# dhansmair/flamingo-mini

Measured on AMD Instinct MI355X. Metric: images/sec (fwd+bwd) flamingo-mini bs=32, higher is better.
Workload: dtype bf16

## Files before the change

### flamingo-mini_amd/csrc/ff_gemm.hip

```cpp
#include <atomic>
#include <type_traits>
#include "ff_common.h"
#include <stdlib.h>
#include "ff_internal.h"
#include "ff_gemm_tiles.h"

namespace ff {

template <typename T>
FF_DEV void epilogue4(const GemmParams& P, const GemmProblem& pr, int m, int n, float (&v)[4]) {
    typedef __attribute__((ext_vector_type(4))) T vec4;
    const long long off = P.c_map.off(m) + n;
    const bool full = (n + 3 < P.N);
#pragma unroll
    for (int r = 0; r < 4; r++) v[r] *= P.scale;
    auto load4 = [&](const void* base, long long at, float (&o)[4]) {
        const T* p = (const T*)base + at;
        if (full) {
            vec4 t = *(const vec4*)p;
#pragma unroll
            for (int r = 0; r < 4; r++) o[r] = to_f32(t[r]);
        } else {
#pragma unroll
            for (int r = 0; r < 4; r++) o[r] = (n + r < P.N) ? to_f32(p[r]) : 0.f;
// ... 1057 lines not shown
    if (dtype == FF_DTYPE_BF16)
        return std::max(plan_bf16(M, N, K, nz, 0, 0, 0).split, plan_bf16(M, N, K, nz, 0, 0, 1).split);
    const long long tiles = (long long)cdiv(M, kFBM) * cdiv(N, kFBM) * nz;
    if (tiles >= 128 || K < 1024) return 1;
    int s = (int)(256 / tiles);
    s = std::min(s, K / 512);
    s = std::min(s, 16);
    return std::max(s, 1);
}

size_t gemm_workspace_bytes(int dtype, int M, int N, int K, int nz, int split_k) {
    if (split_k <= 0) split_k = gemm_pick_split(dtype, M, N, K, nz);
    return split_k > 1 ? (size_t)split_k * nz * M * N * sizeof(float) : 0;
}

int gemm_launch(GemmParams P, int dtype, void* workspace, size_t ws_bytes, hipStream_t st, int* leave_partial) {
    if (leave_partial) *leave_partial = 1;
    FF_CHECK(P.M > 0 && P.N > 0 && P.K > 0 && P.nz >= 1 && P.nz <= kGemmMaxZ, FF_ERR_SHAPE, "gemm: bad shape M=%d N=%d K=%d nz=%d",
             P.M, P.N, P.K, P.nz);
    P.tile = kFBM;
    if (dtype == FF_DTYPE_BF16) {
        const TilePlan plan = plan_bf16(P.M, P.N, P.K, P.nz, P.split_k, P.a_layout, P.b_layout, P.force_tile);
        P.tile = plan.tile;
        P.split_k = plan.split;
    } else if (P.split_k <= 0) P.split_k = gemm_pick_split(dtype, P.M, P.N, P.K, P.nz);
    const int kq = dtype == FF_DTYPE_BF16 ? kBK : kFBK;
    P.k_per_split = cdiv(cdiv(P.K, P.split_k), kq) * kq;
    P.split_k = cdiv(P.K, P.k_per_split);
    P.partial = nullptr;
    if (P.split_k > 1) {
        const size_t need = gemm_workspace_bytes(dtype, P.M, P.N, P.K, P.nz, P.split_k);
        FF_CHECK(workspace && ws_bytes >= need, FF_ERR_WORKSPACE, "gemm split-K workspace: need %zu have %zu", need, ws_bytes);
        FF_CHECK(P.N % 4 == 0, FF_ERR_UNSUPPORTED, "gemm split-K needs N %% 4 == 0 (N=%d)", P.N);
        P.partial = (float*)workspace;
    }
    {
        const int tm_edge = dtype == FF_DTYPE_BF16 ? (P.tile == 256128 || P.tile == 256256 ? 256 : P.tile == 128 || P.tile == 128160 || P.tile == 128002 ? 128 : P.tile == 3264 || P.tile == 3216 ? 32 : 64) : kFBM;
        const int tn_edge = dtype == FF_DTYPE_BF16 ? (P.tile == 3216 ? 16 : P.tile == 64 || P.tile == 64002 || P.tile == 3264 ? 64 : P.tile == 128160 ? 160 : P.tile == 256256 ? 256 : 128) : kFBM;
        const int tiles_m = cdiv(P.M, tm_edge), tiles_n = cdiv(P.N, tn_edge);
        double best = 1e300;
        P.xcd_ms = 1; P.xcd_ns = 1;
        for (int ms = 1; ms <= 8; ms *= 2) {
            const int ns = 8 / ms;
            if (ms > tiles_m || ns > tiles_n) continue;
            const double cost = (double)P.M / ms + (double)P.N / ns;
            if (cost < best) { best = cost; P.xcd_ms = ms; P.xcd_ns = ns; }
        }
        static const int disable = env_int("FF_GEMM_XCD2D", 1) == 0;
        if (disable) { P.xcd_ms = 1; P.xcd_ns = 1; }
    }
    const int vec = dtype == FF_DTYPE_BF16 ? 8 : 4;
    auto map_ok = [&](const RowMap& m) { return m.ld % vec == 0 && (m.rows_per_seg <= 0 || m.seg_stride % vec == 0); };
    const int a_contig = P.a_layout == 0 ? P.K : P.M, b_contig = P.b_layout == 0 ? P.K : P.N;
    P.a_vec_ok = map_ok(P.a_map) && a_contig % vec == 0;
    P.b_vec_ok = map_ok(P.b_map) && b_contig % vec == 0;
    for (int z = 0; z < P.nz; z++) {
        P.a_vec_ok = P.a_vec_ok && ((uintptr_t)P.p[z].A % 16 == 0);
        P.b_vec_ok = P.b_vec_ok && ((uintptr_t)P.p[z].B % 16 == 0);
    }
    P.c_vec8 = P.N % vec == 0 && map_ok(P.c_map) && map_ok(P.r_map);
    for (int z = 0; z < P.nz; z++)
        P.c_vec8 = P.c_vec8 && ((uintptr_t)P.p[z].C | (uintptr_t)P.p[z].aux_out | (uintptr_t)P.p[z].aux_in | (uintptr_t)P.p[z].residual) % 16 == 0;
    int rc;
    const int prof_id = prof_begin(P, dtype, P.tile, st);
    if (dtype == FF_DTYPE_BF16) {
        FF_CHECK(P.a_vec_ok && P.b_vec_ok, FF_ERR_UNSUPPORTED,
                 "bf16 gemm needs 16-byte aligned operands with contiguous dims %% 8 == 0 (M=%d N=%d K=%d)", P.M, P.N, P.K);
        FF_CHECK(P.N % 4 == 0 && P.c_map.ld % 4 == 0, FF_ERR_UNSUPPORTED, "bf16 gemm needs N %% 4 == 0 (N=%d)", P.N);
        auto span_ok = [&](const RowMap& m, int rows, int contig) {
            const long long last = (m.rows_per_seg > 0 ? (long long)((rows - 1) / m.rows_per_seg) * m.seg_stride + (long long)((rows - 1) % m.rows_per_seg) * m.ld
                                                      : (long long)(rows - 1) * m.ld) + contig;
            return last < (1LL << 30);
        };
        FF_CHECK(span_ok(P.a_map, P.a_layout == 0 ? P.M : P.K, a_contig) && span_ok(P.b_map, P.b_layout == 0 ? P.N : P.K, b_contig),
                 FF_ERR_UNSUPPORTED, "bf16 gemm operands must span < 2^30 elements (M=%d N=%d K=%d)", P.M, P.N, P.K);
        rc = run_bf16_dma(P, st);
    } else {
        rc = dispatch_f32(P, st);
    }
    prof_end(prof_id, st);
    FF_TRY(rc);
    if (P.split_k > 1 && leave_partial && P.nz == 1 && P.scale == 1.f && P.act < 0 && P.act_bwd < 0 && !P.p[0].aux_out && !P.p[0].gate &&
        !P.p[0].residual) {
        *leave_partial = P.split_k;
        return FF_OK;
    }
    if (P.split_k > 1) {
        const long long total = (long long)P.nz * P.M * ((P.N + 7) / 8);
        FF_CHECK(total < (1LL << 31), FF_ERR_UNSUPPORTED, "gemm split-K output too large (M=%d N=%d nz=%d)", P.M, P.N, P.nz);
        const int grid = (int)((total + 255) / 256);
        if (dtype == FF_DTYPE_BF16) hipLaunchKernelGGL(gemm_splitk_epilogue_kernel<bf16>, dim3(grid), dim3(256), 0, st, P);
        else hipLaunchKernelGGL(gemm_splitk_epilogue_kernel<float>, dim3(grid), dim3(256), 0, st, P);
        FF_TRY(check_launch("gemm_splitk_epilogue"));
    }
    return FF_OK;
}

}

#ifdef FF_GEMM_TIMELINE
extern "C" int ff_debug_timeline_read(unsigned long long* out, int n_blocks) {
    return (int)hipMemcpyFromSymbol(out, HIP_SYMBOL(ff::g_timeline), sizeof(unsigned long long) * 8 * n_blocks);
}
#endif

extern "C" size_t ff_gemm_workspace_bytes(const ff_gemm_desc* d) {
    int split = d->split_k;
    if (split <= 0 && d->tile > 0 && d->dtype == FF_DTYPE_BF16) split = ff::plan_bf16(d->M, d->N, d->K, 1, 0, d->a_layout, d->b_layout, d->tile).split;
    return ff::gemm_workspace_bytes(d->dtype, d->M, d->N, d->K, 1, split);
}

extern "C" int ff_gemm(const ff_gemm_desc* d, const void* A, const void* B, void* C, void* aux_out, const void* aux_in,
                       const void* residual, const void* gate, void* workspace, size_t workspace_bytes, ff_stream_t stream) {
    using namespace ff;
    FF_CHECK(d && A && B && C, FF_ERR_SHAPE, "ff_gemm: null argument");
    FF_CHECK(d->dtype == FF_DTYPE_F32 || d->dtype == FF_DTYPE_BF16, FF_ERR_UNSUPPORTED, "ff_gemm: dtype %d", d->dtype);
    FF_CHECK(d->act_bwd < 0 || aux_in, FF_ERR_SHAPE, "ff_gemm: act_bwd needs aux_in");
    GemmParams P = {};
    P.M = d->M; P.N = d->N; P.K = d->K;
    P.a_layout = d->a_layout; P.b_layout = d->b_layout;
// ... 56 lines not shown
```

### flamingo-mini_amd/csrc/ff_loss.hip

```cpp
#include "ff_common.h"
#include "ff_internal.h"

namespace ff {

template <typename T, typename F>
FF_DEV void for_row_vectors(const T* row, int V, F&& f) {
    constexpr int N = Vec<T>::N;
    int head = (int)(((16u - (unsigned)((unsigned long long)row & 15u)) & 15u) / sizeof(T));
    head = head < V ? head : V;
    const int nvec = (V - head) / N, tail0 = head + nvec * N;
    if ((int)threadIdx.x < head) f((int)threadIdx.x, to_f32(row[threadIdx.x]));
    for (int v = threadIdx.x; v < nvec; v += 256) {
        float x[N];
        Vec<T>::load(row + head + v * N, x);
#pragma unroll
        for (int e = 0; e < N; e++) f(head + v * N + e, x[e]);
    }
    for (int c = tail0 + threadIdx.x; c < V; c += 256) f(c, to_f32(row[c]));
}

template <typename T>
__global__ __launch_bounds__(256) void shifted_ce_fwd_kernel(int L, int V, const T* __restrict__ logits, const long long* __restrict__ labels,
                                                             long long ignore_index, float* __restrict__ loss_row, float* __restrict__ lse) {
    __shared__ float sm[4], ss[4];
// ... 5 lines not shown
        if (x > m) { s = s * __expf(m - x) + 1.f; m = x; }
        else s += __expf(x - m);
    });
#pragma unroll
    for (int o = 32; o > 0; o >>= 1) {
        const float m2 = __shfl_xor(m, o, 64), s2 = __shfl_xor(s, o, 64);
        const float mn = fmaxf(m, m2);
        s = (m == -INFINITY ? 0.f : s * __expf(m - mn)) + (m2 == -INFINITY ? 0.f : s2 * __expf(m2 - mn));
        m = mn;
    }
    const int w = threadIdx.x >> 6;
    if ((threadIdx.x & 63) == 0) { sm[w] = m; ss[w] = s; }
    __syncthreads();
    if (threadIdx.x == 0) {
        float M = fmaxf(fmaxf(sm[0], sm[1]), fmaxf(sm[2], sm[3])), S = 0.f;
        for (int k = 0; k < 4; k++) S += ss[k] * __expf(sm[k] - M);
        const float l = M + logf(S);
        lse[r] = l;
        const long long tgt = labels[(long long)b * L + i + 1];
        loss_row[r] = tgt == ignore_index ? 0.f : ((tgt < 0 || tgt >= V) ? __builtin_nanf("") : l - to_f32(row[tgt]));
    }
}

template <typename T>
__global__ __launch_bounds__(256) void shifted_ce_bwd_kernel(int L, int V, const T* __restrict__ logits, const long long* __restrict__ labels,
                                                             long long ignore_index, const float* __restrict__ lse, const float* __restrict__ g,
                                                             T* __restrict__ dlogits) {
    pin_args(L, V, logits, labels, ignore_index, lse, g, dlogits);
    const int b = blockIdx.x / L, i = blockIdx.x - b * L;
    const long long off = ((long long)b * L + i) * V;
    constexpr int N = Vec<T>::N;
    const T* row = logits + off;
    T* drow = dlogits + off;
    const bool last = i == L - 1;
    const int r = b * (L - 1) + i;
    const long long tgt = last ? -1 : labels[(long long)b * L + i + 1];
    const float gr = (last || tgt == ignore_index) ? 0.f : ((tgt < 0 || tgt >= V) ? __builtin_nanf("") : g[r]), l = last ? 0.f : lse[r];
    auto dval = [&](int c, float x) { return gr == 0.f ? 0.f : (__expf(x - l) - (c == tgt ? 1.f : 0.f)) * gr; };
    int head = (int)(((16u - (unsigned)((unsigned long long)row & 15u)) & 15u) / sizeof(T));
    head = head < V ? head : V;
    const int nvec = (V - head) / N, tail0 = head + nvec * N;
    if ((int)threadIdx.x < head) drow[threadIdx.x] = from_f32<T>(dval(threadIdx.x, to_f32(row[threadIdx.x])));
    for (int v = threadIdx.x; v < nvec; v += 256) {
        const int c0 = head + v * N;
        float x[N];
        Vec<T>::load(row + c0, x);
#pragma unroll
        for (int e = 0; e < N; e++) x[e] = dval(c0 + e, x[e]);
        Vec<T>::store(drow + c0, x);
    }
    for (int c = tail0 + threadIdx.x; c < V; c += 256) drow[c] = from_f32<T>(dval(c, to_f32(row[c])));
}

}

extern "C" int ff_shifted_ce_fwd(int dtype, int batch, int seq, int vocab, const void* logits, const long long* labels, long long ignore_index,
                                 float* loss_row, float* lse, ff_stream_t stream) {
    using namespace ff;
    FF_CHECK(batch > 0 && seq > 1 && vocab > 0 && logits && labels && loss_row && lse, FF_ERR_SHAPE, "ff_shifted_ce_fwd: bad arguments");
    const dim3 grid(batch * (seq - 1));
    if (dtype == FF_DTYPE_BF16) shifted_ce_fwd_kernel<bf16><<<grid, dim3(256), 0, (hipStream_t)stream>>>(seq, vocab, (const bf16*)logits, labels, ignore_index, loss_row, lse);
    else if (dtype == FF_DTYPE_F32) shifted_ce_fwd_kernel<float><<<grid, dim3(256), 0, (hipStream_t)stream>>>(seq, vocab, (const float*)logits, labels, ignore_index, loss_row, lse);
    else FF_CHECK(false, FF_ERR_UNSUPPORTED, "ff_shifted_ce_fwd: dtype %d", dtype);
    return check_launch("shifted_ce_fwd");
}

extern "C" int ff_shifted_ce_bwd(int dtype, int batch, int seq, int vocab, const void* logits, const long long* labels, long long ignore_index,
                                 const float* lse, const float* grad_row, void* dlogits, ff_stream_t stream) {
    using namespace ff;
    FF_CHECK(batch > 0 && seq > 1 && vocab > 0 && logits && labels && lse && grad_row && dlogits, FF_ERR_SHAPE, "ff_shifted_ce_bwd: bad arguments");
    FF_CHECK((((unsigned long long)logits ^ (unsigned long long)dlogits) & 15u) == 0, FF_ERR_UNSUPPORTED, "ff_shifted_ce_bwd: logits and dlogits must share their 16-byte alignment phase");
    const dim3 grid(batch * seq);
    if (dtype == FF_DTYPE_BF16) shifted_ce_bwd_kernel<bf16><<<grid, dim3(256), 0, (hipStream_t)stream>>>(seq, vocab, (const bf16*)logits, labels, ignore_index, lse, grad_row, (bf16*)dlogits);
    else if (dtype == FF_DTYPE_F32) shifted_ce_bwd_kernel<float><<<grid, dim3(256), 0, (hipStream_t)stream>>>(seq, vocab, (const float*)logits, labels, ignore_index, lse, grad_row, (float*)dlogits);
    else FF_CHECK(false, FF_ERR_UNSUPPORTED, "ff_shifted_ce_bwd: dtype %d", dtype);
    return check_launch("shifted_ce_bwd");
}
```

### flamingo-mini_amd/ffi.py

```python
from __future__ import annotations

import ctypes as C
import os
from typing import Optional, Sequence

import torch

PKG_DIR = os.path.dirname(os.path.abspath(__file__))
_which = os.environ.get("FLAMINGO_FUSION_LIB", "")
LIB_PATH = os.path.join(PKG_DIR, "libflamingo_fusion_debug.so") if _which == "debug" else (_which or os.path.join(PKG_DIR, "libflamingo_fusion.so"))
ABI_VERSION = 6

FF_OK = 0
DTYPE_F32, DTYPE_BF16 = 0, 1
ACT_NONE, ACT_GELU, ACT_SQRELU, ACT_RELU = -1, 0, 1, 2
ACTS = {"gelu": ACT_GELU, "sqrelu": ACT_SQRELU, "relu": ACT_RELU}
ATTN_DENSE, ATTN_MEDIA = 0, 1
RESAMPLER_GLOBAL_PARAMS, RESAMPLER_LAYER_PARAMS, XATTN_PARAMS = 4, 12, 11
WGRAD_GROUP_MAX = 12


class FusionLibraryError(RuntimeError):
    pass

# ... 55 lines not shown

class XattnDesc(C.Structure):
    _fields_ = [("dtype", C.c_int), ("batch", C.c_int), ("n_tokens", C.c_int), ("dim", C.c_int), ("dim_visual", C.c_int),
                ("n_media", C.c_int), ("n_visual", C.c_int), ("heads", C.c_int), ("dim_head", C.c_int), ("ff_mult", C.c_int),
                ("act", C.c_int), ("tt_stride", C.c_int), ("tt_offset", C.c_int), ("cached_k", Strides), ("cached_v", Strides),
                ("sync", C.c_void_p)]


_P, _SZ, _I = C.c_void_p, C.c_size_t, C.c_int
_SIGNATURES = {
    "ff_version": (_I, []),
    "ff_arch": (C.c_char_p, []),
    "ff_last_error": (C.c_char_p, []),
    "ff_gemm_workspace_bytes": (_SZ, [C.POINTER(GemmDesc)]),
    "ff_gemm": (_I, [C.POINTER(GemmDesc), _P, _P, _P, _P, _P, _P, _P, _P, _SZ, _P]),
    "ff_gemm_profile_enable": (_I, [_I]),
    "ff_gemm_profile_read": (_I, [C.POINTER(GemmProfileRecord), _I]),
    "ff_gemm_plan": (_I, [C.POINTER(GemmDesc), C.POINTER(_I), C.POINTER(_I), C.POINTER(_I)]),
    "ff_layernorm_fwd": (_I, [C.POINTER(LnDesc), _P, _P, _P, _P, _P, _P, _P, _P]),
    "ff_layernorm_bwd_workspace_bytes": (_SZ, [C.POINTER(LnDesc)]),
    "ff_layernorm_bwd": (_I, [C.POINTER(LnDesc), _P, _P, _P, _P, _P, _P, _P, _P, _P, _P, _P, _SZ, _P]),
    "ff_rows_reduce_workspace_bytes": (_SZ, [C.POINTER(ReduceDesc)]),
    "ff_rows_reduce": (_I, [C.POINTER(ReduceDesc), _P, _P, _P, _SZ, _P]),
    "ff_gate_grad_workspace_bytes": (_SZ, [_I, _I]),
    "ff_gate_grad": (_I, [_I, _I, _I, _P, _P, _P, _P, _P, _SZ, _P]),
    "ff_text_time": (_I, [_I, _I, _P, _I, _P, _P]),
    "ff_attention_fwd": (_I, [C.POINTER(AttnDesc), _P, _P, _P, _P, _P, _P, _P]),
    "ff_attention_bwd_workspace_bytes": (_SZ, [C.POINTER(AttnDesc)]),
    "ff_attention_bwd": (_I, [C.POINTER(AttnDesc), _P, _P, _P, _P, _P, _P, _P, _P, _P, _P, _P, _SZ, _P]),
    "ff_resampler_saved_bytes": (_SZ, [C.POINTER(ResamplerDesc)]),
    "ff_resampler_scratch_bytes": (_SZ, [C.POINTER(ResamplerDesc)]),
    "ff_resampler_fwd": (_I, [C.POINTER(ResamplerDesc), _P, _P, _P, _P, _SZ, _P, _SZ, _P]),
    "ff_resampler_bwd": (_I, [C.POINTER(ResamplerDesc), _P, _P, _P, _P, _SZ, _P, _P, _P, _SZ, _P]),
    "ff_resampler_prologue_saved_bytes": (_SZ, [C.POINTER(ResamplerDesc)]),
    "ff_resampler_layer_saved_bytes": (_SZ, [C.POINTER(ResamplerDesc)]),
    "ff_resampler_layer_scratch_bytes": (_SZ, [C.POINTER(ResamplerDesc)]),
    "ff_resampler_epilogue_saved_bytes": (_SZ, [C.POINTER(ResamplerDesc)]),
    "ff_resampler_prologue_fwd": (_I, [C.POINTER(ResamplerDesc), _P, _P, _P, _SZ, _P]),
    "ff_resampler_layer_fwd": (_I, [C.POINTER(ResamplerDesc), _P, _P, _P, _SZ, _P, _I, _P, _P, _P, _SZ, _P, _SZ, _P]),
    "ff_resampler_epilogue_fwd": (_I, [C.POINTER(ResamplerDesc), _P, _P, _P, _P, _P, _SZ, _P]),
    "ff_resampler_epilogue_bwd": (_I, [C.POINTER(ResamplerDesc), _P, _P, _P, _P, _SZ, _P, _P, _P, _P, _SZ, _P]),
    "ff_resampler_layer_bwd": (_I, [C.POINTER(ResamplerDesc), _P, _P, _P, _SZ, _P, _I, _P, _P, _P, _SZ, _P, _P, _P, _I, _P, _SZ, _P]),
    "ff_resampler_prologue_bwd": (_I, [C.POINTER(ResamplerDesc), _P, _P, _P, _P, _P, _SZ, _P]),
    "ff_xattn_sync_bytes": (_SZ, []),
    "ff_xattn_sync_status": (_I, [_P, _P]),
    "ff_xattn_saved_bytes": (_SZ, [C.POINTER(XattnDesc)]),
    "ff_xattn_scratch_bytes": (_SZ, [C.POINTER(XattnDesc)]),
    "ff_xattn_kv_offset": (_SZ, [C.POINTER(XattnDesc)]),
    "ff_xattn_block_fwd": (_I, [C.POINTER(XattnDesc), _P, _P, _P, _P, _P, _P, _P, _P, _SZ, _P, _SZ, _P]),
    "ff_quick_gelu_fwd": (_I, [_I, C.c_longlong, _P, _P, _P]),
    "ff_quick_gelu_bwd": (_I, [_I, C.c_longlong, _P, _P, _P, _P]),
    "ff_shifted_ce_fwd": (_I, [_I, _I, _I, _I, _P, _P, C.c_longlong, _P, _P, _P]),
    "ff_shifted_ce_bwd": (_I, [_I, _I, _I, _I, _P, _P, C.c_longlong, _P, _P, _P, _P]),
    "ff_adamw_step": (_I, [C.POINTER(AdamWDesc), _P, _P, _P, _P, _P, _P]),
    "ff_adamw_step_mixed": (_I, [C.POINTER(AdamWDesc), _I, _P, _P, _P, _P, _P, _P, _P, _P]),
    "ff_adamw_step_clipped": (_I, [C.POINTER(AdamWDesc), _I, _P, _P, _P, _P, _P, _P, _P, _P, _P]),
    "ff_grad_sumsq_partials": (C.c_longlong, [_I, _P]),
    "ff_grad_sumsq": (_I, [_I, _I, _P, _P, C.c_float, _P, C.c_longlong, _P]),
    "ff_grad_sumsq_reduce": (_I, [_P, C.c_longlong, _P, _I, _P]),
    "ff_grad_clip_coef": (_I, [_P, C.c_float, _P, _P, _P]),
    "ff_scale_grads": (_I, [_I, _I, _P, _P, _P, _P]),
    "ff_grad_accumulate": (_I, [_I, _I, _P, _P, _P, C.c_float, _I, _P]),
    "ff_adamw_step_acc": (_I, [C.POINTER(AdamWDesc), _I, _P, _P, _P, _P, _P, _P, _P, _P, _P]),
    "ff_xattn_block_bwd_kv": (_I, [C.POINTER(XattnDesc), _P, _P, _P, _P, _P, _P, _P, _SZ, _P, _P, _P, _P, _SZ, _P]),
    "ff_kv_project_workspace_bytes": (_SZ, [C.POINTER(KvProjDesc), _I]),
    "ff_kv_project_fwd": (_I, [C.POINTER(KvProjDesc), _P, _P, _P, _P, _SZ, _P]),
    "ff_kv_project_bwd": (_I, [C.POINTER(KvProjDesc), _P, _P, _P, _P, _P, _P, _SZ, _P]),
    "ff_xattn_wgrad_stash_bytes": (_SZ, [C.POINTER(XattnDesc)]),
    "ff_xattn_wgrad_workspace_bytes": (_SZ, [C.POINTER(XattnDesc)]),
    "ff_xattn_block_bwd_kv_data": (_I, [C.POINTER(XattnDesc), _P, _P, _P, _P, _P, _P, _P, _SZ, _P, _P, _P, _P, _SZ, _P, _SZ, _P]),
    "ff_xattn_wgrad_grouped": (_I, [C.POINTER(XattnDesc), _I, _P, _P, _SZ, _P, _SZ, _P, _P, _P, _SZ, _P]),
    "ff_xattn_block_bwd": (_I, [C.POINTER(XattnDesc), _P, _P, _P, _P, _P, _P, _SZ, _P, _P, _P, _P, _SZ, _P]),
}
EXPORTED_SYMBOLS = tuple(_SIGNATURES)

_lib: Optional[C.CDLL] = None


def lib() -> C.CDLL:
    global _lib
    if _lib is not None:
        return _lib
    if not os.path.exists(LIB_PATH):
        raise FusionLibraryError(
            f"{LIB_PATH} is missing: build it with `python -m flamingo_mini_amd.build` (needs hipcc, gfx950). "
            "There is no CPU/PyTorch fallback for the fusion path.")
    try:
        handle = C.CDLL(LIB_PATH)
    except OSError as e:
        raise FusionLibraryError(f"cannot load {LIB_PATH}: {e}") from e
    for name, (res, args) in _SIGNATURES.items():
        try:
            fn = getattr(handle, name)
        except AttributeError as e:
            raise FusionLibraryError(f"{LIB_PATH} does not export {name}; rebuild it") from e
        fn.restype = res
        fn.argtypes = args
    if handle.ff_version() != ABI_VERSION:
        raise FusionLibraryError(f"ABI mismatch: library {handle.ff_version()} vs binding {ABI_VERSION}; rebuild")
    _lib = handle
    return handle


_TRACE = os.environ.get("FF_TRACE", "0") == "1"


# ... 41 lines not shown
```

### flamingo-mini_amd/functional.py

```python
from __future__ import annotations

from typing import Callable, Optional, Sequence, Tuple

import torch

from . import ffi

_grad_ready_callbacks: list = []


def _new(shape, dtype, device) -> torch.Tensor:
    return torch.empty(shape, dtype=dtype, device=device)


def _new_zeros(shape, dtype, device) -> torch.Tensor:
    return torch.zeros(shape, dtype=dtype, device=device)


def _new_like(t: torch.Tensor, dtype=None) -> torch.Tensor:
    return torch.empty_like(t, dtype=dtype)


def _new_zeros_like(t: torch.Tensor, dtype=None) -> torch.Tensor:
    return torch.zeros_like(t, dtype=dtype)
# ... 678 lines not shown
    @staticmethod
    def forward(ctx, x):
        x = x.contiguous()
        y = _new_like(x)
        ffi.check(ffi.lib().ff_quick_gelu_fwd(ffi.dtype_code(x.dtype), x.numel(), x.data_ptr(), y.data_ptr(), ffi.stream_handle(x.device)),
                  "ff_quick_gelu_fwd")
        ctx.save_for_backward(x)
        return y

    @staticmethod
    def backward(ctx, dy):
        (x,) = ctx.saved_tensors
        dy = dy.contiguous()
        dx = _new_like(x)
        ffi.check(ffi.lib().ff_quick_gelu_bwd(ffi.dtype_code(x.dtype), x.numel(), x.data_ptr(), dy.data_ptr(), dx.data_ptr(),
                                              ffi.stream_handle(x.device)), "ff_quick_gelu_bwd")
        return dx


def quick_gelu(x: torch.Tensor) -> torch.Tensor:
    ffi.require_cuda(x)
    return _QuickGeluFn.apply(x)


class _ShiftedCEFn(torch.autograd.Function):
    @staticmethod
    def forward(ctx, logits, labels, ignore_index):
        lib = ffi.lib()
        logits = logits.contiguous()
        labels = labels.contiguous().to(torch.int64)
        b, L, V = logits.shape
        rows = _new(b * (L - 1), torch.float32, logits.device)
        lse = _new_like(rows)
        ffi.check(lib.ff_shifted_ce_fwd(ffi.dtype_code(logits.dtype), b, L, V, logits.data_ptr(), labels.data_ptr(), ignore_index,
                                        rows.data_ptr(), lse.data_ptr(), ffi.stream_handle(logits.device)), "ff_shifted_ce_fwd")
        ctx.ignore_index = ignore_index
        ctx.save_for_backward(logits, labels, lse)
        return rows

    @staticmethod
    def backward(ctx, grad_rows):
        lib = ffi.lib()
        logits, labels, lse = ctx.saved_tensors
        b, L, V = logits.shape
        dlogits = _new_like(logits)
        g = grad_rows.contiguous().float()
        ffi.check(lib.ff_shifted_ce_bwd(ffi.dtype_code(logits.dtype), b, L, V, logits.data_ptr(), labels.data_ptr(), ctx.ignore_index,
                                        lse.data_ptr(), g.data_ptr(), dlogits.data_ptr(), ffi.stream_handle(logits.device)), "ff_shifted_ce_bwd")
        return dlogits, None, None


def shifted_cross_entropy(logits: torch.Tensor, labels: torch.Tensor, reduction: str = "mean", ignore_index: int = -100) -> torch.Tensor:
    ffi.require_cuda(logits, labels)
    rows = _ShiftedCEFn.apply(logits, labels, ignore_index)
    if reduction == "none":
        return rows
    if reduction == "sum":
        return rows.sum()
    if reduction == "mean":
        count = (labels[..., 1:] != ignore_index).sum()
        return rows.sum() / count
    raise ValueError(f"unknown reduction {reduction}")


def gemm(A, B, *, a_layout=0, b_layout=0, scale=1.0, act=None, act_bwd=None, aux_in=None, residual=None, gate=None,
         want_aux_out=False, split_k=0, tile=0, stages=0):
    lib = ffi.lib()
    ffi.require_cuda(A, B)
    M, K = (A.shape if a_layout == 0 else A.shape[::-1])
    N = B.shape[0] if b_layout == 0 else B.shape[1]
    C_ = _new((M, N), A.dtype, A.device)
    aux_out = _new_like(C_) if want_aux_out else None
    d = ffi.GemmDesc(ffi.dtype_code(A.dtype), M, N, K, a_layout, b_layout, ffi.rowmap(A.stride(0)), ffi.rowmap(B.stride(0)),
                     ffi.rowmap(N), float(scale), ffi.ACTS.get(act, ffi.ACT_NONE), ffi.ACTS.get(act_bwd, ffi.ACT_NONE), split_k, tile, stages)
    ws = _empty_bytes(lib.ff_gemm_workspace_bytes(d), A.device)
    ffi.check(lib.ff_gemm(d, A.data_ptr(), B.data_ptr(), C_.data_ptr(), ffi.ptr(aux_out), ffi.ptr(aux_in), ffi.ptr(residual), ffi.ptr(gate),
                          ws.data_ptr(), ws.numel(), ffi.stream_handle(A.device)), "ff_gemm")
    return (C_, aux_out) if want_aux_out else C_


def layernorm_fwd(x, gamma, beta, add=None, add_rows_per_seg=0, add_div=0, eps=1e-5):
    lib = ffi.lib()
    rows, cols = x.shape
    y = _new_like(x)
    mean = _new(rows, torch.float32, x.device)
    rstd = _new_like(mean)
    d = ffi.LnDesc(ffi.dtype_code(x.dtype), rows, cols, ffi.rowmap(cols), ffi.rowmap(cols), ffi.rowmap(cols), add_rows_per_seg, add_div, eps, 0)
    ffi.check(lib.ff_layernorm_fwd(d, x.data_ptr(), ffi.ptr(add), gamma.data_ptr(), beta.data_ptr(), y.data_ptr(), mean.data_ptr(),
                                   rstd.data_ptr(), ffi.stream_handle(x.device)), "ff_layernorm_fwd")
    return y, mean, rstd


def layernorm_bwd(dy, x, gamma, mean, rstd, add=None, add_rows_per_seg=0, add_div=0, dx_residual=None, eps=1e-5):
    lib = ffi.lib()
    rows, cols = x.shape
    dx = _new_like(x)
    dg, db = _new_like(gamma), _new_like(gamma)
    d = ffi.LnDesc(ffi.dtype_code(x.dtype), rows, cols, ffi.rowmap(cols), ffi.rowmap(cols), ffi.rowmap(cols), add_rows_per_seg, add_div, eps, 1)
    ws = _empty_bytes(lib.ff_layernorm_bwd_workspace_bytes(d), x.device)
    ffi.check(lib.ff_layernorm_bwd(d, dy.data_ptr(), x.data_ptr(), ffi.ptr(add), gamma.data_ptr(), mean.data_ptr(), rstd.data_ptr(),
                                   dx.data_ptr(), ffi.ptr(dx_residual), dg.data_ptr(), db.data_ptr(), ws.data_ptr(), ws.numel(),
                                   ffi.stream_handle(x.device)), "ff_layernorm_bwd")
    return dx, dg, db


def rows_reduce(x, rows_per_batch, rows_per_group):
    lib = ffi.lib()
    rows, cols = x.shape
    out = _new((rows_per_batch // rows_per_group, cols), x.dtype, x.device)
    d = ffi.ReduceDesc(ffi.dtype_code(x.dtype), rows, cols, ffi.rowmap(cols), rows_per_batch, rows_per_group)
    ws = _empty_bytes(lib.ff_rows_reduce_workspace_bytes(d), x.device)
    ffi.check(lib.ff_rows_reduce(d, x.data_ptr(), out.data_ptr(), ws.data_ptr(), ws.numel(), ffi.stream_handle(x.device)), "ff_rows_reduce")
    return out


def gate_grad(a, b, alpha):
    lib = ffi.lib()
    rows, cols = a.shape
    out = _new_like(alpha)
    ws = _empty_bytes(lib.ff_gate_grad_workspace_bytes(rows, cols), a.device)
    ffi.check(lib.ff_gate_grad(ffi.dtype_code(a.dtype), rows, cols, a.data_ptr(), b.data_ptr(), alpha.data_ptr(), out.data_ptr(),
                               ws.data_ptr(), ws.numel(), ffi.stream_handle(a.device)), "ff_gate_grad")
# ... 38 lines not shown
```

### flamingo-mini_amd/modeling_flamingo.py

```python
from __future__ import annotations

import contextlib
import logging
from abc import ABC, abstractmethod
from typing import Any, Dict, List, Optional

import torch
import torch.nn as nn
import torch.nn.functional as TF
from transformers import PreTrainedModel
from transformers.modeling_outputs import CausalLMOutputWithPast

from . import functional as F
from .backbones import load_language_model, load_vision_encoder
from .configuration_flamingo import FlamingoConfig
from .gated_cross_attention import ModifiedLMBlock
from .graphs import _prepared_capture_stream
from .perceiver_resampler import PerceiverResampler
from .utils import get_common_prefix_length


@contextlib.contextmanager
def suppress_model_loading_warnings(suppress: bool = True):
    logger = logging.getLogger("transformers.modeling_utils")
# ... 117 lines not shown
                head_mask=None, inputs_embeds=None, use_cache: bool = False, past_key_values=None, return_dict: bool = True,
                labels=None, loss_reduction: str = "mean", text_time=None, **kwargs) -> CausalLMOutputWithPast:
        assert return_dict, "can only use return_dict=True at the moment!"
        assert (input_ids is None) != (inputs_embeds is None), "you must pass either input_ids or inputs_embeds!"
        ref = input_ids if input_ids is not None else inputs_embeds
        batch_size, seq_length = ref.shape[:2]
        device = ref.device
        xattn_past = None if past_key_values is None else past_key_values[0]
        lm_past = None if past_key_values is None else past_key_values[1]

        if visual_features is None:
            if xattn_past is None and pixel_values is not None:
                assert pixel_values.size(0) == batch_size, "pixel_values must have the same batch size as the textual input!"
                visual_features = self.encode_resample_visuals(pixel_values)
            else:
                visual_features = torch.zeros((batch_size, 1, self.config.resampler_num_latents, self.config.dim_visual),
                                              dtype=self.resampler.latents.dtype, device=device)
        if self.training and (getattr(self.lm, "gradient_checkpointing", False) or any(getattr(m, "gradient_checkpointing", False) for m in self.lm.modules())):
            raise NotImplementedError("activation checkpointing of the language model is not supported by the fused cross-attention hooks: "
                                      "their conditioning (visual features, hoisted K / V) is released when forward() returns. "
                                      "Disable gradient checkpointing (the frozen LM keeps few activations: only the trainable blocks save theirs).")
        if self.training and device.type == "cuda" and not torch.cuda.is_current_stream_capturing():
            F.poll_sync_exchange("FlamingoBaseModel.forward")
        cuts = getattr(self, "_autograd_cuts", None)
        if cuts is not None and xattn_past is None:
            visual_features = cuts.cut(visual_features)
        if text_time is None:
            if media_locations is None:
                media_locations = torch.zeros((batch_size, seq_length), dtype=torch.int, device=device)
            text_time = F.text_time(media_locations)
        hooks = self.get_modified_layers()
        hoisted = None
        if xattn_past is None and self.hoist_kv:
            weights = [h.xattn_block.attn.to_kv.weight for h in hooks]
            cdt = F.autocast_compute_dtype(visual_features)
            if cdt is not None:
                weights = F.autocast_params(weights, cdt)
            vf_cast = visual_features.to(weights[0].dtype)
            step = self.kv_project_group if self.kv_project_group > 0 else len(weights)
            hoisted = [kv for g in range(0, len(weights), step) for kv in F.kv_project(vf_cast, weights[g:g + step])]
        for i, hook in enumerate(hooks):
            hook.condition(visual_features, media_locations, None if xattn_past is None else xattn_past[i], text_time=text_time,
                           hoisted_kv=None if hoisted is None else hoisted[i])

        lm_kwargs = dict(input_ids=input_ids, attention_mask=attention_mask, inputs_embeds=inputs_embeds, use_cache=use_cache,
                         past_key_values=lm_past, return_dict=True, **kwargs)
        if head_mask is not None:
            lm_kwargs["head_mask"] = head_mask
        try:
            out = self.lm(**lm_kwargs)
        finally:
            for hook in hooks:
                hook.condition(None, None)
        logits = self.lm_head(out.last_hidden_state)

        new_xattn_past = [hook.kv_output for hook in hooks] if use_cache else None
        for hook in hooks:
            hook.kv_output = None

        loss = None
        if labels is not None:
            if logits.is_cuda and logits.dtype in (torch.float32, torch.bfloat16) and logits.ndim == 3 and seq_length > 1:
                loss = F.shifted_cross_entropy(logits, labels, reduction=loss_reduction)
            else:
                flat = logits[..., :-1, :].contiguous().view(-1, logits.size(-1))
                if flat.dtype in (torch.bfloat16, torch.float16):
                    flat = flat.float()
                loss = TF.cross_entropy(flat, labels[..., 1:].contiguous().view(-1), reduction=loss_reduction)

        return CausalLMOutputWithPast(
            loss=loss, logits=logits,
            past_key_values=(tuple(new_xattn_past), out.past_key_values) if use_cache else None,
            hidden_states=getattr(out, "hidden_states", None), attentions=getattr(out, "attentions", None))


class FlamingoGPT2(FlamingoBaseModel):
    _tied_weights_keys = {"lm_head.weight": "lm.wte.weight"}

    def __init__(self, config: FlamingoConfig):
        assert config.lm.startswith("gpt")
        super().__init__(config)
        base_lm = load_language_model(config)
        assert config.dim == base_lm.config.n_embd, \
            f"specified {config.dim=} in FlamingoConfig, but {config.lm} has hidden size={base_lm.config.n_embd}"
        _add_eoc_row(base_lm)
        self.lm = base_lm.transformer
        self.lm_head = base_lm.lm_head
        self._init_layers(self.lm.h)
        self.post_init()

    def get_modified_layers(self):
        return [layer for layer in self.lm.h if isinstance(layer, ModifiedLMBlock)]


class FlamingoOPT(FlamingoBaseModel):
    _tied_weights_keys = {"lm_head.weight": "lm.decoder.embed_tokens.weight"}

    def __init__(self, config: FlamingoConfig):
        assert config.lm.startswith("facebook/opt")
        super().__init__(config)
        base_lm = load_language_model(config)
        assert config.dim == base_lm.config.hidden_size, \
            f"specified {config.dim=} in FlamingoConfig, but {config.lm} has hidden size={base_lm.config.hidden_size}"
        _add_eoc_row(base_lm)
        self.lm = base_lm.model
        self.lm_head = base_lm.lm_head
        self._init_layers(self.lm.decoder.layers)
        self.post_init()

    def get_modified_layers(self):
        return [layer for layer in self.lm.decoder.layers if isinstance(layer, ModifiedLMBlock)]


import weakref
# ... 408 lines not shown
```

### include/flamingo_fusion.h

```cpp
#ifndef FLAMINGO_FUSION_H
#define FLAMINGO_FUSION_H

#include <stddef.h>

#ifdef __cplusplus
extern "C" {
#endif
#if defined(__GNUC__) || defined(__clang__)
#pragma GCC visibility push(default)
#endif

typedef struct ihipStream_t* ff_stream_t;

enum { FF_OK = 0, FF_ERR_SHAPE = -1, FF_ERR_UNSUPPORTED = -2, FF_ERR_WORKSPACE = -3, FF_ERR_LAUNCH = -4 };
enum { FF_DTYPE_F32 = 0, FF_DTYPE_BF16 = 1 };
enum { FF_ACT_NONE = -1, FF_ACT_GELU = 0, FF_ACT_SQRELU = 1, FF_ACT_RELU = 2 };

int ff_version(void);
const char* ff_arch(void);
const char* ff_last_error(void);

typedef struct ff_rowmap {
    long long ld;
    long long seg_stride;
// ... 154 lines not shown
} ff_kvproj_desc;
size_t ff_kv_project_workspace_bytes(const ff_kvproj_desc* d, int with_dvisual_features);
int ff_kv_project_fwd(const ff_kvproj_desc* d, const void* visual_features, const void* const* w_kv, void* const* kv_out,
                      void* workspace, size_t workspace_bytes, ff_stream_t stream);
int ff_kv_project_bwd(const ff_kvproj_desc* d, const void* visual_features, const void* const* w_kv, const void* const* dkv,
                      void* const* dw_kv, void* dvisual_features, void* workspace, size_t workspace_bytes, ff_stream_t stream);
int ff_xattn_block_bwd_kv(const ff_xattn_desc* d, const void* y, const void* k, const void* v, const int* text_time,
                          const void* const* params, const void* dy_out, const void* saved, size_t saved_bytes, void* const* grads,
                          void* dy, void* dkv, void* scratch, size_t scratch_bytes, ff_stream_t stream);

#define FF_WGRAD_GROUP_MAX 12
size_t ff_xattn_wgrad_stash_bytes(const ff_xattn_desc* d);
size_t ff_xattn_wgrad_workspace_bytes(const ff_xattn_desc* d);
int ff_xattn_block_bwd_kv_data(const ff_xattn_desc* d, const void* y, const void* k, const void* v, const int* text_time,
                               const void* const* params, const void* dy_out, const void* saved, size_t saved_bytes, void* const* grads,
                               void* dy, void* dkv, void* stash, size_t stash_bytes, void* scratch, size_t scratch_bytes, ff_stream_t stream);
int ff_xattn_wgrad_grouped(const ff_xattn_desc* d, int n_blocks, const void* const* dy_out, const void* const* saved, size_t saved_bytes,
                           const void* const* stash, size_t stash_bytes, const void* const* params, void* const* grads, void* workspace,
                           size_t workspace_bytes, ff_stream_t stream);

typedef struct ff_adamw_desc {
    int dtype;
    int n_tensors;
    int step;
    float lr, beta1, beta2, eps, weight_decay, grad_scale;
    const float* step_dev;
} ff_adamw_desc;
int ff_adamw_step(const ff_adamw_desc* d, void* const* params, const void* const* grads, void* const* exp_avg,
                  void* const* exp_avg_sq, const long long* numels, ff_stream_t stream);
int ff_adamw_step_mixed(const ff_adamw_desc* d, int state_dtype, void* const* params, const void* const* grads, void* const* exp_avg,
                        void* const* exp_avg_sq, float* const* master, const float* lr_dev, const long long* numels, ff_stream_t stream);
int ff_adamw_step_clipped(const ff_adamw_desc* d, int state_dtype, void* const* params, const void* const* grads, void* const* exp_avg,
                          void* const* exp_avg_sq, float* const* master, const float* lr_dev, const float* grad_coef, const long long* numels,
                          ff_stream_t stream);

long long ff_grad_sumsq_partials(int n_tensors, const long long* numels);
int ff_grad_sumsq(int dtype, int n_tensors, const void* const* grads, const long long* numels, float scale, float* partials,
                  long long n_partials, ff_stream_t stream);
int ff_grad_sumsq_reduce(const float* partials, long long n_partials, double* sum, int accumulate, ff_stream_t stream);
int ff_grad_clip_coef(const double* sum, float max_norm, float* norm, float* coef, ff_stream_t stream);
int ff_scale_grads(int dtype, int n_tensors, void* const* grads, const long long* numels, const float* coef, ff_stream_t stream);

int ff_grad_accumulate(int dtype, int n_tensors, const void* const* grads, float* const* acc, const long long* numels, float scale,
                       int overwrite, ff_stream_t stream);
int ff_adamw_step_acc(const ff_adamw_desc* d, int state_dtype, void* const* params, const float* const* grads32, void* const* exp_avg,
                      void* const* exp_avg_sq, float* const* master, const float* lr_dev, const float* grad_coef, const long long* numels,
                      ff_stream_t stream);


int ff_shifted_ce_fwd(int dtype, int batch, int seq, int vocab, const void* logits, const long long* labels, long long ignore_index,
                      float* loss_row, float* lse, ff_stream_t stream);
int ff_shifted_ce_bwd(int dtype, int batch, int seq, int vocab, const void* logits, const long long* labels, long long ignore_index,
                      const float* lse, const float* grad_row, void* dlogits, ff_stream_t stream);

int ff_quick_gelu_fwd(int dtype, long long n, const void* x, void* y, ff_stream_t stream);
int ff_quick_gelu_bwd(int dtype, long long n, const void* x, const void* dy, void* dx, ff_stream_t stream);

#if defined(__GNUC__) || defined(__clang__)
#pragma GCC visibility pop
#endif
#ifdef __cplusplus
}
#endif
#endif
```

Baseline: 780.3.

## Fuse lm_head projection with shifted cross-entropy and use padded dlogits for dgrad

Adds an autograd function that computes the lm_head logits and the shifted CE loss together, then in backward writes dlogits into a row buffer padded to 64 columns. The hidden-state gradient uses the custom bf16 GEMM with split-K directly on the padded buffer, and the GEMM vector check is relaxed so K-major rows padded to the vector width are accepted. This removes the separate CE backward pass through autograd and enables the vectorized GEMM path when the vocab size is not a multiple of 8. In exchange it allocates a padded gradient buffer, takes a strided view for the weight gradient, and adds a new kernel with packed unaligned loads.

```diff
diff --git a/flamingo-mini_amd/csrc/ff_gemm.hip b/flamingo-mini_amd/csrc/ff_gemm.hip
--- a/flamingo-mini_amd/csrc/ff_gemm.hip
+++ b/flamingo-mini_amd/csrc/ff_gemm.hip
@@ -1133,8 +1133,11 @@
     const int vec = dtype == FF_DTYPE_BF16 ? 8 : 4;
     auto map_ok = [&](const RowMap& m) { return m.ld % vec == 0 && (m.rows_per_seg <= 0 || m.seg_stride % vec == 0); };
     const int a_contig = P.a_layout == 0 ? P.K : P.M, b_contig = P.b_layout == 0 ? P.K : P.N;
-    P.a_vec_ok = map_ok(P.a_map) && a_contig % vec == 0;
-    P.b_vec_ok = map_ok(P.b_map) && b_contig % vec == 0;
+    auto contig_ok = [&](const RowMap& m, int layout, int contig) {
+        return contig % vec == 0 || (layout == 0 && m.ld >= (long long)cdiv(contig, vec) * vec);
+    };
+    P.a_vec_ok = map_ok(P.a_map) && contig_ok(P.a_map, P.a_layout, a_contig);
+    P.b_vec_ok = map_ok(P.b_map) && contig_ok(P.b_map, P.b_layout, b_contig);
     for (int z = 0; z < P.nz; z++) {
         P.a_vec_ok = P.a_vec_ok && ((uintptr_t)P.p[z].A % 16 == 0);
         P.b_vec_ok = P.b_vec_ok && ((uintptr_t)P.p[z].B % 16 == 0);
@@ -1146,7 +1149,7 @@
     const int prof_id = prof_begin(P, dtype, P.tile, st);
     if (dtype == FF_DTYPE_BF16) {
         FF_CHECK(P.a_vec_ok && P.b_vec_ok, FF_ERR_UNSUPPORTED,
-                 "bf16 gemm needs 16-byte aligned operands with contiguous dims %% 8 == 0 (M=%d N=%d K=%d)", P.M, P.N, P.K);
+                 "bf16 gemm needs 16-byte aligned operands with contiguous dims %% 8 == 0, or K-major rows padded to that (M=%d N=%d K=%d)", P.M, P.N, P.K);
         FF_CHECK(P.N % 4 == 0 && P.c_map.ld % 4 == 0, FF_ERR_UNSUPPORTED, "bf16 gemm needs N %% 4 == 0 (N=%d)", P.N);
         auto span_ok = [&](const RowMap& m, int rows, int contig) {
             const long long last = (m.rows_per_seg > 0 ? (long long)((rows - 1) / m.rows_per_seg) * m.seg_stride + (long long)((rows - 1) % m.rows_per_seg) * m.ld
diff --git a/flamingo-mini_amd/csrc/ff_loss.hip b/flamingo-mini_amd/csrc/ff_loss.hip
--- a/flamingo-mini_amd/csrc/ff_loss.hip
+++ b/flamingo-mini_amd/csrc/ff_loss.hip
@@ -81,6 +81,42 @@
     for (int c = tail0 + threadIdx.x; c < V; c += 256) drow[c] = from_f32<T>(dval(c, to_f32(row[c])));
 }
 
+template <int SA> struct __attribute__((packed, aligned(SA))) RawChunk { unsigned char b[16]; };
+template <typename T, int SA>
+__global__ __launch_bounds__(256) void shifted_ce_bwd_ld_kernel(int L, int V, long long ld, const T* __restrict__ logits, const long long* __restrict__ labels,
+                                                                long long ignore_index, const float* __restrict__ lse, const float* __restrict__ g,
+                                                                T* __restrict__ dlogits) {
+    pin_args(L, V, ld, logits, labels, ignore_index, lse, g, dlogits);
+    const int b = blockIdx.x / L, i = blockIdx.x - b * L;
+    constexpr int N = Vec<T>::N;
+    const T* row = logits + ((long long)b * L + i) * V;
+    T* drow = dlogits + (long long)blockIdx.x * ld;
+    const bool last = i == L - 1;
+    const int r = b * (L - 1) + i;
+    const long long tgt = last ? -1 : labels[(long long)b * L + i + 1];
+    const float gr = (last || tgt == ignore_index) ? 0.f : ((tgt < 0 || tgt >= V) ? __builtin_nanf("") : g[r]), l = last ? 0.f : lse[r];
+    auto dval = [&](int c, float x) { return gr == 0.f ? 0.f : (__expf(x - l) - (c == tgt ? 1.f : 0.f)) * gr; };
+    const int nfull = V / N, nvec = (int)(ld / N);
+    for (int v = threadIdx.x; v < nvec; v += 256) {
+        const int c0 = v * N;
+        float x[N];
+        if (gr == 0.f) {
+#pragma unroll
+            for (int e = 0; e < N; e++) x[e] = 0.f;
+        } else if (v < nfull) {
+            const RawChunk<SA> raw = *(const RawChunk<SA>*)(row + c0);
+            T t[N];
+            __builtin_memcpy(t, &raw, 16);
+#pragma unroll
+            for (int e = 0; e < N; e++) x[e] = dval(c0 + e, to_f32(t[e]));
+        } else {
+#pragma unroll
+            for (int e = 0; e < N; e++) x[e] = c0 + e < V ? dval(c0 + e, to_f32(row[c0 + e])) : 0.f;
+        }
+        Vec<T>::store(drow + c0, x);
+    }
+}
+
 }
 
 extern "C" int ff_shifted_ce_fwd(int dtype, int batch, int seq, int vocab, const void* logits, const long long* labels, long long ignore_index,
@@ -105,3 +141,22 @@
     else FF_CHECK(false, FF_ERR_UNSUPPORTED, "ff_shifted_ce_bwd: dtype %d", dtype);
     return check_launch("shifted_ce_bwd");
 }
+
+extern "C" int ff_shifted_ce_bwd_ld(int dtype, int batch, int seq, int vocab, const void* logits, const long long* labels, long long ignore_index,
+                                    const float* lse, const float* grad_row, void* dlogits, long long ld_out, ff_stream_t stream) {
+    using namespace ff;
+    FF_CHECK(batch > 0 && seq > 1 && vocab > 0 && logits && labels && lse && grad_row && dlogits, FF_ERR_SHAPE, "ff_shifted_ce_bwd_ld: bad arguments");
+    FF_CHECK(dtype == FF_DTYPE_BF16 || dtype == FF_DTYPE_F32, FF_ERR_UNSUPPORTED, "ff_shifted_ce_bwd_ld: dtype %d", dtype);
+    const int es = dtype == FF_DTYPE_BF16 ? 2 : 4, vec = 16 / es;
+    FF_CHECK(ld_out >= vocab && ld_out % vec == 0 && ld_out < (1LL << 31), FF_ERR_SHAPE, "ff_shifted_ce_bwd_ld: ld_out %lld must be >= vocab %d and a multiple of %d",
+             ld_out, vocab, vec);
+    FF_CHECK((unsigned long long)dlogits % 16 == 0 && (unsigned long long)logits % es == 0, FF_ERR_UNSUPPORTED,
+             "ff_shifted_ce_bwd_ld: dlogits must be 16-byte aligned (and logits element-aligned)");
+    const bool a4 = ((unsigned long long)logits | ((unsigned long long)vocab * es)) % 4 == 0;
+    const dim3 grid(batch * seq);
+    const hipStream_t st = (hipStream_t)stream;
+    if (dtype == FF_DTYPE_F32) shifted_ce_bwd_ld_kernel<float, 4><<<grid, dim3(256), 0, st>>>(seq, vocab, ld_out, (const float*)logits, labels, ignore_index, lse, grad_row, (float*)dlogits);
+    else if (a4) shifted_ce_bwd_ld_kernel<bf16, 4><<<grid, dim3(256), 0, st>>>(seq, vocab, ld_out, (const bf16*)logits, labels, ignore_index, lse, grad_row, (bf16*)dlogits);
+    else shifted_ce_bwd_ld_kernel<bf16, 2><<<grid, dim3(256), 0, st>>>(seq, vocab, ld_out, (const bf16*)logits, labels, ignore_index, lse, grad_row, (bf16*)dlogits);
+    return check_launch("shifted_ce_bwd_ld");
+}
diff --git a/flamingo-mini_amd/ffi.py b/flamingo-mini_amd/ffi.py
--- a/flamingo-mini_amd/ffi.py
+++ b/flamingo-mini_amd/ffi.py
@@ -131,6 +131,7 @@
     "ff_quick_gelu_bwd": (_I, [_I, C.c_longlong, _P, _P, _P, _P]),
     "ff_shifted_ce_fwd": (_I, [_I, _I, _I, _I, _P, _P, C.c_longlong, _P, _P, _P]),
     "ff_shifted_ce_bwd": (_I, [_I, _I, _I, _I, _P, _P, C.c_longlong, _P, _P, _P, _P]),
+    "ff_shifted_ce_bwd_ld": (_I, [_I, _I, _I, _I, _P, _P, C.c_longlong, _P, _P, _P, C.c_longlong, _P]),
     "ff_adamw_step": (_I, [C.POINTER(AdamWDesc), _P, _P, _P, _P, _P, _P]),
     "ff_adamw_step_mixed": (_I, [C.POINTER(AdamWDesc), _I, _P, _P, _P, _P, _P, _P, _P, _P]),
     "ff_adamw_step_clipped": (_I, [C.POINTER(AdamWDesc), _I, _P, _P, _P, _P, _P, _P, _P, _P, _P]),
diff --git a/flamingo-mini_amd/functional.py b/flamingo-mini_amd/functional.py
--- a/flamingo-mini_amd/functional.py
+++ b/flamingo-mini_amd/functional.py
@@ -754,7 +754,10 @@
 
 def shifted_cross_entropy(logits: torch.Tensor, labels: torch.Tensor, reduction: str = "mean", ignore_index: int = -100) -> torch.Tensor:
     ffi.require_cuda(logits, labels)
-    rows = _ShiftedCEFn.apply(logits, labels, ignore_index)
+    return _reduce_loss_rows(_ShiftedCEFn.apply(logits, labels, ignore_index), labels, reduction, ignore_index)
+
+
+def _reduce_loss_rows(rows: torch.Tensor, labels: torch.Tensor, reduction: str, ignore_index: int) -> torch.Tensor:
     if reduction == "none":
         return rows
     if reduction == "sum":
@@ -765,11 +768,82 @@
     raise ValueError(f"unknown reduction {reduction}")
 
 
+LM_HEAD_LD_ALIGN = 64
+
+
+def _lm_head_dgrad_split(M: int, N: int, K: int) -> int:
+    tiles = -(-M // 128) * -(-N // 128)
+    split = min(512 // tiles, 8, K // (64 * 64))
+    return split if split >= 2 else 0
+
+
+class _LmHeadLossFn(torch.autograd.Function):
+    @staticmethod
+    def forward(ctx, hidden, weight, labels, ignore_index):
+        lib = ffi.lib()
+        ctx.set_materialize_grads(False)
+        logits = torch.nn.functional.linear(hidden, weight)
+        labels = labels.contiguous().to(torch.int64)
+        b, L, V = logits.shape
+        rows = _new(b * (L - 1), torch.float32, logits.device)
+        lse = _new_like(rows)
+        ffi.check(lib.ff_shifted_ce_fwd(ffi.dtype_code(logits.dtype), b, L, V, logits.data_ptr(), labels.data_ptr(), ignore_index,
+                                        rows.data_ptr(), lse.data_ptr(), ffi.stream_handle(logits.device)), "ff_shifted_ce_fwd")
+        ctx.ignore_index = ignore_index
+        ctx.save_for_backward(hidden, weight, logits, labels, lse)
+        return logits, rows
+
+    @staticmethod
+    def backward(ctx, grad_logits, grad_rows):
+        lib = ffi.lib()
+        hidden, weight, logits, labels, lse = ctx.saved_tensors
+        if grad_logits is None and grad_rows is None:
+            return None, None, None, None
+        b, L, V = logits.shape
+        M, dim = b * L, weight.shape[1]
+        dev, stream = logits.device, ffi.stream_handle(logits.device)
+        ld = (V + LM_HEAD_LD_ALIGN - 1) // LM_HEAD_LD_ALIGN * LM_HEAD_LD_ALIGN
+        dlogits = _new((M, ld), logits.dtype, dev)
+        g = grad_rows.contiguous().float() if grad_rows is not None else torch.zeros(b * (L - 1), dtype=torch.float32, device=dev)
+        ffi.check(lib.ff_shifted_ce_bwd_ld(ffi.dtype_code(logits.dtype), b, L, V, logits.data_ptr(), labels.data_ptr(), ctx.ignore_index,
+                                           lse.data_ptr(), g.data_ptr(), dlogits.data_ptr(), ld, stream), "ff_shifted_ce_bwd_ld")
+        valid = dlogits[:, :V]
+        if grad_logits is not None:
+            valid += grad_logits.reshape(M, V)
+        dhidden = dweight = None
+        if ctx.needs_input_grad[0]:
+            dh = _new((M, dim), logits.dtype, dev)
+            d = ffi.GemmDesc(ffi.dtype_code(logits.dtype), M, dim, V, 0, 1, ffi.rowmap(ld), ffi.rowmap(weight.stride(0)), ffi.rowmap(dim),
+                             1.0, ffi.ACT_NONE, ffi.ACT_NONE, _lm_head_dgrad_split(M, dim, V), 0, 0)
+            ws = _empty_bytes(lib.ff_gemm_workspace_bytes(d), dev)
+            ffi.check(lib.ff_gemm(d, dlogits.data_ptr(), weight.data_ptr(), dh.data_ptr(), None, None, None, None, ws.data_ptr(), ws.numel(), stream),
+                      "ff_gemm(lm_head d hidden)")
+            dhidden = dh.view(hidden.shape)
+        if ctx.needs_input_grad[1]:
+            dweight = valid.t().mm(hidden.reshape(M, dim))
+        return dhidden, dweight, None, None
+
+
+def lm_head_loss_supported(hidden: torch.Tensor, weight: torch.Tensor) -> bool:
+    return (hidden.is_cuda and weight.is_cuda and hidden.dtype == torch.bfloat16 and weight.dtype == torch.bfloat16
+            and autocast_compute_dtype(hidden) is None and hidden.ndim == 3 and hidden.shape[1] > 1 and weight.ndim == 2
+            and hidden.is_contiguous() and weight.is_contiguous() and weight.shape[1] == hidden.shape[2] and weight.shape[1] % 8 == 0
+            and hidden.data_ptr() % 16 == 0 and weight.data_ptr() % 16 == 0)
+
+
+def lm_head_shifted_cross_entropy(hidden: torch.Tensor, weight: torch.Tensor, labels: torch.Tensor, reduction: str = "mean",
+                                  ignore_index: int = -100) -> Tuple[torch.Tensor, torch.Tensor]:
+    ffi.require_cuda(hidden, weight, labels)
+    logits, rows = _LmHeadLossFn.apply(hidden, weight, labels, ignore_index)
+    return logits, _reduce_loss_rows(rows, labels, reduction, ignore_index)
+
+
 def gemm(A, B, *, a_layout=0, b_layout=0, scale=1.0, act=None, act_bwd=None, aux_in=None, residual=None, gate=None,
-         want_aux_out=False, split_k=0, tile=0, stages=0):
+         want_aux_out=False, split_k=0, tile=0, stages=0, K=None):
     lib = ffi.lib()
     ffi.require_cuda(A, B)
-    M, K = (A.shape if a_layout == 0 else A.shape[::-1])
+    M, k_full = (A.shape if a_layout == 0 else A.shape[::-1])
+    K = k_full if K is None else int(K)
     N = B.shape[0] if b_layout == 0 else B.shape[1]
     C_ = _new((M, N), A.dtype, A.device)
     aux_out = _new_like(C_) if want_aux_out else None
diff --git a/flamingo-mini_amd/modeling_flamingo.py b/flamingo-mini_amd/modeling_flamingo.py
--- a/flamingo-mini_amd/modeling_flamingo.py
+++ b/flamingo-mini_amd/modeling_flamingo.py
@@ -193,14 +193,20 @@
         finally:
             for hook in hooks:
                 hook.condition(None, None)
-        logits = self.lm_head(out.last_hidden_state)
+        hidden = out.last_hidden_state
+        loss = None
+        head = self.lm_head
+        if (labels is not None and isinstance(head, nn.Linear) and head.bias is None and not head._forward_hooks and not head._forward_pre_hooks
+                and F.lm_head_loss_supported(hidden, head.weight)):
+            logits, loss = F.lm_head_shifted_cross_entropy(hidden, head.weight, labels, reduction=loss_reduction)
+        else:
+            logits = head(hidden)
 
         new_xattn_past = [hook.kv_output for hook in hooks] if use_cache else None
         for hook in hooks:
             hook.kv_output = None
 
-        loss = None
-        if labels is not None:
+        if labels is not None and loss is None:
             if logits.is_cuda and logits.dtype in (torch.float32, torch.bfloat16) and logits.ndim == 3 and seq_length > 1:
                 loss = F.shifted_cross_entropy(logits, labels, reduction=loss_reduction)
             else:
diff --git a/include/flamingo_fusion.h b/include/flamingo_fusion.h
--- a/include/flamingo_fusion.h
+++ b/include/flamingo_fusion.h
@@ -230,6 +230,8 @@
                       float* loss_row, float* lse, ff_stream_t stream);
 int ff_shifted_ce_bwd(int dtype, int batch, int seq, int vocab, const void* logits, const long long* labels, long long ignore_index,
                       const float* lse, const float* grad_row, void* dlogits, ff_stream_t stream);
+int ff_shifted_ce_bwd_ld(int dtype, int batch, int seq, int vocab, const void* logits, const long long* labels, long long ignore_index,
+                         const float* lse, const float* grad_row, void* dlogits, long long ld_out, ff_stream_t stream);
 
 int ff_quick_gelu_fwd(int dtype, long long n, const void* x, void* y, ff_stream_t stream);
 int ff_quick_gelu_bwd(int dtype, long long n, const void* x, const void* dy, void* dx, ff_stream_t stream);
```

Measured after the change: 786.1, median of 6. About the same (+0.7%).
